# ladnlav/OFDM-course

Hardware: AMD Instinct MI355X
Metric: OFDM sym/s full Task-5 RX (Nfft=2048, 64-QAM, OMP) (higher is better)
Workload: dtype f32; 1 GPU; M: Nfft=2048 Tg=256 N_carrier=512 comb=4 (128 pilots, K=128) 64QAM OMP(6 taps) Noise(20 dB) -> 6-tap channel (the reference's order), frames of 14 symbols; frames_per_gpu=20480

## Files before the change

### ofdm-course_amd/csrc/chain_fast_core.hpp

```cpp
#pragma once
#include <cstdlib>
#include <map>
#include <utility>
#include <vector>
#include <type_traits>

#include "demap_core.hpp"
#include "fft_core.hpp"

namespace ofdm {

constexpr int FAST_MAXT = 32;

__device__ __forceinline__ void wave_sync() {
  __builtin_amdgcn_fence(__ATOMIC_RELEASE, "wavefront");
  __builtin_amdgcn_wave_barrier();
  __builtin_amdgcn_fence(__ATOMIC_ACQUIRE, "wavefront");
}

constexpr int WAVE_LDS_ELEMS = 512 + 64;

constexpr int WAVE_TW_ELEMS = 2 * 7 * 64;

template <typename T, int NW>
__device__ __forceinline__ void wave_tw_fill(cx<T>* __restrict__ twl, const cx<T>* __restrict__ tw) {
  for (int i = threadIdx.x; i < WAVE_TW_ELEMS; i += 64 * NW) {
    const int pass = i / 448, r = i - pass * 448, t = r / 64 + 1, l = r & 63;
    twl[i] = pass == 0 ? tw[(t * (l & 7) * 8) * NW] : tw[(t * l) * NW];
  }
}

template <typename T>
__device__ __forceinline__ void dft8_first2(cx<T> (&v)[8]) {
  const T h = T(0.70710678118654752440084436210485);
  const cx<T> a0 = v[0] + v[4], a1 = v[1] + v[5], a2 = v[2] + v[6], a3 = v[3] + v[7];
  const cx<T> b0 = v[0] - v[4];
  cx<T> b1 = v[1] - v[5], b2 = v[2] - v[6], b3 = v[3] - v[7];
  b1 = mk<T>((b1.x + b1.y) * h, (b1.y - b1.x) * h);
  b2 = mk<T>(b2.y, -b2.x);
  b3 = mk<T>((b3.y - b3.x) * h, (-b3.x - b3.y) * h);
  v[0] = (a0 + a2) + (a1 + a3);
  v[1] = (b0 + b2) + (b1 + b3);
}

template <int STRIDE, bool ASM>
__device__ __forceinline__ void lds_read8(cx<float> (&v)[8], const cx<float>* base) {
  if constexpr (ASM) {
    const unsigned a = (unsigned)(uintptr_t)base;
    unsigned long long r0, r1, r2, r3, r4, r5, r6, r7;
    asm volatile(
        "ds_read_b64 %0, %8 offset:%9\n\t"
        "ds_read_b64 %1, %8 offset:%10\n\t"
        "ds_read_b64 %2, %8 offset:%11\n\t"
        "ds_read_b64 %3, %8 offset:%12\n\t"
        "ds_read_b64 %4, %8 offset:%13\n\t"
        "ds_read_b64 %5, %8 offset:%14\n\t"
        "ds_read_b64 %6, %8 offset:%15\n\t"
        "ds_read_b64 %7, %8 offset:%16\n\t"
        "s_waitcnt lgkmcnt(0)"
        : "=&v"(r0), "=&v"(r1), "=&v"(r2), "=&v"(r3), "=&v"(r4), "=&v"(r5), "=&v"(r6), "=&v"(r7)
        : "v"(a), "n"(0 * STRIDE * 8), "n"(1 * STRIDE * 8), "n"(2 * STRIDE * 8), "n"(3 * STRIDE * 8),
          "n"(4 * STRIDE * 8), "n"(5 * STRIDE * 8), "n"(6 * STRIDE * 8), "n"(7 * STRIDE * 8)
        : "memory");
    const unsigned long long r[8] = {r0, r1, r2, r3, r4, r5, r6, r7};
#pragma unroll
    for (int e = 0; e < 8; ++e) {
      v[e].x = __uint_as_float((unsigned)r[e]);
      v[e].y = __uint_as_float((unsigned)(r[e] >> 32));
    }
  } else {
#pragma unroll
    for (int e = 0; e < 8; ++e) v[e] = base[STRIDE * e];
  }
}
template <int STRIDE, bool ASM>
__device__ __forceinline__ void lds_read8(cx<double> (&v)[8], const cx<double>* base) {
#pragma unroll
  for (int e = 0; e < 8; ++e) v[e] = base[STRIDE * e];
}

template <typename T, bool PRUNE2, bool TWB_REG = true, bool ASMRD = false>
__device__ __forceinline__ void wave_fft512(cx<T> (&v)[8], int lane, const cx<T> (&twb)[7],
                                            const cx<T>* __restrict__ twl, cx<T>* __restrict__ lw) {
  cx<T>* const sa = lw + 72 * (lane >> 3) + (lane & 3) + 36 * ((lane >> 2) & 1);
  cx<T>* const ga1 = lw + ((lane >> 3) & 3) + 36 * (lane >> 5) + 4 * (lane & 7);
  cx<T>* const sb = lw + 72 * (lane >> 3) + (lane & 7);
  cx<T>* const ga2 = lw + lane;
  dft8<T, false>(v[0], v[1], v[2], v[3], v[4], v[5], v[6], v[7]);
#pragma unroll
  for (int t = 0; t < 8; ++t) sa[4 * t] = v[t];
  wave_sync();
  lds_read8<72, ASMRD>(v, ga1);
  wave_sync();
#pragma unroll
  for (int t = 1; t < 8; ++t) v[t] = v[t] * (TWB_REG ? twb[t - 1] : twl[(t - 1) * 64 + lane]);
  dft8<T, false>(v[0], v[1], v[2], v[3], v[4], v[5], v[6], v[7]);
#pragma unroll
  for (int t = 0; t < 8; ++t) sb[8 * t] = v[t];
  wave_sync();
  lds_read8<72, ASMRD>(v, ga2);
  wave_sync();
#pragma unroll
  for (int t = 1; t < 8; ++t) v[t] = v[t] * twl[448 + (t - 1) * 64 + lane];
  if constexpr (PRUNE2) dft8_first2<T>(v);
  else dft8<T, false>(v[0], v[1], v[2], v[3], v[4], v[5], v[6], v[7]);
}

template <typename T, int NW>
struct DifTw {
  cx<T> w[NW > 1 ? (8 / NW) * (NW - 1) : 1];
};

template <typename T, int NW>
__device__ __forceinline__ void dif_tw_init(DifTw<T, NW>& d, int gid, const cx<T>* __restrict__ tw) {
  if constexpr (NW > 1) {
    constexpr int BPT = 8 / NW;
#pragma unroll
    for (int b = 0; b < BPT; ++b)
#pragma unroll
      for (int s = 1; s < NW; ++s) d.w[b * (NW - 1) + (s - 1)] = tw[(gid * BPT + b) * s];
  }
}

template <typename T, int NW>
__device__ __forceinline__ void frame_load(cx<T> (&v)[8], const cx<T>* __restrict__ src ,
                                           int gid, int lane) {
  if constexpr (NW == 1) {
#pragma unroll
    for (int e = 0; e < 8; ++e) v[e] = nt_load(src + lane + 64 * e);
  } else {
    constexpr int BPT = 8 / NW;
#pragma unroll
    for (int t = 0; t < NW; ++t)
#pragma unroll
      for (int b = 0; b < BPT; ++b) v[b * NW + t] = nt_load(src + gid * BPT + b + 512 * t);
  }
}

template <typename T, int NW>
__device__ __forceinline__ void dif_stage(cx<T> (&v)[8], const DifTw<T, NW>& d) {
  if constexpr (NW > 1) {
// ... 415 lines not shown
  const float* d_sb_w;
  const int32_t* d_sb_c0;
  void** ws_v;
  int64_t* ws_v_frames;
  void** ws_h;
  void** ws_x;
  int64_t* ws_x_elems;
  int data_mod4;
  uint32_t descr;
};

template <typename T>
int fast_params_prepare(const FastPlanView& pv, const void* tw, int64_t n_frames, FastParams<T>& P);
template <typename T>
int omp_batch_run(const FastParams<T>& P, int64_t n_frames);

template <typename T>
int eq_demap_run(const FastPlanView& pv, const FastParams<T>& P, const cx<T>* xk, int x_stride, bool hext, int64_t n_frames,
                 void* bits, const void* ref, void* errs, void* h_out, void* idx_out, const double* fine_est, int time_desync,
                 int freq_desync, int mer_skip = 0,
                 double* mer_sums = nullptr );

int mmse_build_operator(const c64* h, int64_t n_h, double snr_db, const int32_t* pilot_loc, int np, int n_carrier,
                        int m_pad, std::vector<c64>& wt, std::vector<c64>* mt_out = nullptr, int np_pad = 0,
                        std::vector<double>* sop_out = nullptr);
void mmse_band_spline(const std::vector<double>& sop, int nc, int np, std::vector<float>& w, std::vector<int32_t>& c0, int& bw, int& span);
int spline_band_run(const float* sb_w, const int32_t* sb_c0, int bw, int span, const void* v, void* hout, int np, int n_carrier,
                    int64_t n_frames);
bool mmse_factored_usable(int np, int np_pad);
int mmse_factored_run(const void* mt, int np_pad, const float* sb_w, const int32_t* sb_c0, int bw, int span, const void* y, void* v,
                      void* hout, int np, int n_carrier, int64_t n_frames);
template <typename T>
int mmse_apply_run(const void* wt, const void* y, void* hout, int np, int m_pad, int n_carrier, int64_t n_frames);

template <typename T>
inline int mmse_stage_run(const FastPlanView& pv, const FastParams<T>& P, int64_t n_frames) {
  if constexpr (std::is_same<T, float>::value) {
    if (pv.d_mt && mmse_factored_usable(pv.np, pv.np_pad)) {
      int64_t& cap = *pv.ws_v_frames;
      if (!*pv.ws_v || cap < n_frames) {
        OFDM_HIP(hipStreamSynchronize(ctx().stream));
        if (*pv.ws_v) { (void)hipFree(*pv.ws_v); *pv.ws_v = nullptr; }
        OFDM_HIP(hipMalloc(pv.ws_v, sizeof(cx<float>) * (size_t)pv.np * n_frames));
        cap = n_frames;
      }
      return mmse_factored_run(pv.d_mt, pv.np_pad, pv.d_sb_w, pv.d_sb_c0, pv.sb_bw, pv.sb_span, P.ypil, *pv.ws_v, *pv.ws_h, pv.np,
                               pv.n_carrier, n_frames);
    }
  }
  return mmse_apply_run<T>(pv.d_wt, P.ypil, *pv.ws_h, pv.np, pv.m_pad, pv.n_carrier, n_frames);
}

bool chain_wave_supported(const FastPlanView& pv);
int chain_wave_symbols_run(const FastPlanView& pv, const FastParams<float>& P, const void* rx, int64_t n_frames, void* bits,
                           const void* ref, void* errs, void* h_out, void* idx_out, double* mer = nullptr );

bool chain_coop_supported(const FastPlanView& pv);
int chain_coop_symbols_run(const FastPlanView& pv, const FastParams<float>& P, const void* rx, int64_t n_frames, void* bits,
                           const void* ref, void* errs, void* h_out, void* idx_out, double* mer = nullptr );

template <typename T>
int pilot_omp_run(const FastParams<T>& P, int nfft, bool prune2, int lg_up, const void* rx, int64_t n_frames);

}
```

### ofdm-course_amd/csrc/ofdm_chain_fast.hip

```cpp
#include "chain_fast_core.hpp"
#include "omp_wave_core.hpp"

namespace ofdm {

template <typename T, int NW, bool PRUNE2>
__global__ __launch_bounds__(64 * NW, sizeof(T) == 4 ? (PRUNE2 ? 4 : 3) : 2) void rx_pilot_kernel(FastParams<T> P, const cx<T>* __restrict__ rx,
                                                           int64_t n_frames) {
  constexpr int N = 512 * NW;
  constexpr int NOUT = PRUNE2 ? 2 : 8;
  __shared__ cx<T> lwv[NW * WAVE_LDS_ELEMS];
  __shared__ cx<T> twl[WAVE_TW_ELEMS];
  cx<T>* const ex = lwv;
  const int wave = threadIdx.x >> 6, lane = threadIdx.x & 63, gid = threadIdx.x;
  DifTw<T, NW> dt;
  wave_tw_fill<T, NW>(twl, P.tw);
  dif_tw_init<T, NW>(dt, gid, P.tw);
  cx<T> twb[7];
#pragma unroll
  for (int t = 1; t < 8; ++t) twb[t - 1] = P.tw[(t * (lane & 7) * 8) * NW];
  __syncthreads();
  int kk[NOUT], pp[NOUT];
#pragma unroll
  for (int t = 0; t < NOUT; ++t) {
    kk[t] = NW * (lane + 64 * t) + wave;
// ... 338 lines not shown
  P.tap_idx = (int32_t*)*pv.ws_tapidx; P.tap_x = (c64*)*pv.ws_tapx;
  const bool mmse = pv.d_wt != nullptr;
  if (mmse && !*pv.ws_h) {
    OFDM_HIP(hipStreamSynchronize(ctx().stream));
    OFDM_HIP(hipMalloc(pv.ws_h, sizeof(cx<T>) * (size_t)pv.n_carrier * *pv.ws_frames));
  }
  P.h_in = mmse ? (const cx<T>*)*pv.ws_h : nullptr;
  P.descr = pv.descr;
  return OFDM_OK;
}
template int fast_params_prepare<float>(const FastPlanView&, const void*, int64_t, FastParams<float>&);
template int fast_params_prepare<double>(const FastPlanView&, const void*, int64_t, FastParams<double>&);

template <typename T>
int omp_batch_run(const FastParams<T>& P, int64_t n_frames) {
  hipStream_t st = ctx().stream;
  const bool by_fft = P.comb_m == 2048 && P.np <= 2048 && P.k_atoms <= 2048 && !getenv("OFDM_OMP_NO_FFT");
  const OmpLayout lay = omp_layout<T>(P.np, P.k_atoms, P.taps, by_fft ? fft_lds_elems(2048) : 0);
  OFDM_ARG(lay.total <= 150 * 1024, "rx_chain_task5: OMP stage needs %u bytes of LDS", lay.total);
  const unsigned grid = cdiv_u(n_frames, 4 * lay.fpw);
  const bool mfma = std::is_same<T, float>::value && (P.k_atoms % 16 == 0) && (P.np % 4 == 0) && !getenv("OFDM_OMP_NO_MFMA");
  auto launch = [&](auto kern, const void* twm) -> int {
    OFDM_HIP(hipFuncSetAttribute((const void*)kern, hipFuncAttributeMaxDynamicSharedMemorySize, (int)lay.total));
    hipLaunchKernelGGL(kern, dim3(grid), dim3(256), lay.total, st, P, lay, n_frames, (const cx<T>*)twm);
    return OFDM_OK;
  };
  if (by_fft) {
    const void* twm = nullptr;
    OFDM_TRY(get_twiddles(2048, std::is_same<T, double>::value, &twm));
    OFDM_TRY(launch(omp_batch_kernel<T, false, 2048>, twm));
  } else if (mfma) {
    if constexpr (std::is_same<T, float>::value) OFDM_TRY(launch(omp_batch_kernel<T, true>, nullptr));
  } else {
    OFDM_TRY(launch(omp_batch_kernel<T, false>, nullptr));
  }
  return check_launch("omp_batch_kernel");
}
template int omp_batch_run<float>(const FastParams<float>&, int64_t);
template int omp_batch_run<double>(const FastParams<double>&, int64_t);

template <typename T, int NW, bool PRUNE2>
static int launch_fast(const FastPlanView& pv, const void* tw, const void* rx, int64_t n_frames, void* bits,
                       const void* ref, void* errs, void* h_out, void* idx_out, double* mer) {
  FastParams<T> P;
  OFDM_TRY(fast_params_prepare<T>(pv, tw, n_frames, P));
  const bool mmse = pv.d_wt != nullptr;
  DemapTable<T> tab;
  fill_demap_table<T>(*pv.dict, *pv.cinfo, tab);
  const int ncu = ctx().num_cu;
  hipStream_t st = ctx().stream;
  if (pv.ev) OFDM_HIP(hipEventRecord(pv.ev[0], st));
  const bool fused = !mmse && pv.comb_lg_up >= 0 && pv.taps <= OMP_RT && pv.k_atoms <= 512 && !getenv("OFDM_FAST_UNFUSED");
  if (pv.fused_out) *pv.fused_out = fused ? 1 : 0;
  if (fused) {
    OFDM_TRY(pilot_omp_run<T>(P, 512 * NW, PRUNE2, pv.comb_lg_up, rx, n_frames));
    if (pv.ev) OFDM_HIP(hipEventRecord(pv.ev[1], st));
  } else {
    {
      const unsigned grid = (unsigned)std::min<int64_t>(n_frames, (int64_t)ncu * std::max(1, 16 / NW));
      hipLaunchKernelGGL((rx_pilot_kernel<T, NW, PRUNE2>), dim3(grid), dim3(64 * NW), 0, st, P, (const cx<T>*)rx, n_frames);
      OFDM_TRY(check_launch("rx_pilot_kernel"));
    }
    if (pv.ev) OFDM_HIP(hipEventRecord(pv.ev[1], st));
    if (mmse) {
      OFDM_TRY(mmse_stage_run<T>(pv, P, n_frames));
    } else {
      OFDM_TRY(omp_batch_run<T>(P, n_frames));
    }
  }
  if (pv.ev && !fused) OFDM_HIP(hipEventRecord(pv.ev[2], st));
  if constexpr (std::is_same<T, float>::value && NW == 4 && PRUNE2) {
    if (chain_wave_supported(pv) && !(mer && getenv("OFDM_WAVE_EXACT_SLICER"))) {
      OFDM_TRY(chain_wave_symbols_run(pv, P, rx, n_frames, bits, ref, errs, h_out, idx_out, mer));
      if (pv.ev) OFDM_HIP(hipEventRecord(pv.ev[3], st));
      return OFDM_OK;
    }
  }
  {
    constexpr int N = 512 * NW;
    const size_t dyn = sizeof(cx<T>) * ((size_t)NW * WAVE_LDS_ELEMS + WAVE_TW_ELEMS) +
                       (((size_t)pv.nd * pv.n_symb + 31) & ~size_t(31));
    OFDM_ARG(dyn <= 150 * 1024, "rx_chain_task5: symbol stage needs %zu bytes of LDS", dyn);
    auto launch = [&](auto kern, auto... mer_arg) -> int {
      int per_cu = resident_blocks_per_cu((const void*)kern, 64 * NW, dyn);
      if (const char* e = getenv("OFDM_FAST_WG_PER_CU")) per_cu = std::max(1, atoi(e));
      const unsigned grid = (unsigned)std::min<int64_t>(n_frames, (int64_t)ncu * per_cu);
      hipLaunchKernelGGL(kern, dim3(grid), dim3(64 * NW), dyn, st, P, (const cx<T>*)rx, n_frames, (uint32_t*)bits,
                         (const uint32_t*)ref, (uint32_t*)errs, (cx<T>*)h_out, (int32_t*)idx_out, tab, mer_arg...);
      return OFDM_OK;
    };
    const int ba = pv.cinfo->kind == 1 ? pv.cinfo->bits_per_axis : 0;
    if (mer) {
      const MerSums ms{mer};
      switch (ba) {
        case 2: OFDM_TRY(mmse ? launch(rx_symbols_kernel<T, NW, PRUNE2, 2, true, MerSums>, ms)
                              : launch(rx_symbols_kernel<T, NW, PRUNE2, 2, false, MerSums>, ms)); break;
        case 3: OFDM_TRY(mmse ? launch(rx_symbols_kernel<T, NW, PRUNE2, 3, true, MerSums>, ms)
                              : launch(rx_symbols_kernel<T, NW, PRUNE2, 3, false, MerSums>, ms)); break;
        case 4: OFDM_TRY(mmse ? launch(rx_symbols_kernel<T, NW, PRUNE2, 4, true, MerSums>, ms)
                              : launch(rx_symbols_kernel<T, NW, PRUNE2, 4, false, MerSums>, ms)); break;
        default: OFDM_TRY(mmse ? launch(rx_symbols_kernel<T, NW, PRUNE2, 0, true, MerSums>, ms)
                               : launch(rx_symbols_kernel<T, NW, PRUNE2, 0, false, MerSums>, ms)); break;
      }
    } else if (mmse) {
      switch (ba) {
        case 2: OFDM_TRY(launch(rx_symbols_kernel<T, NW, PRUNE2, 2, true>)); break;
        case 3: OFDM_TRY(launch(rx_symbols_kernel<T, NW, PRUNE2, 3, true>)); break;
        case 4: OFDM_TRY(launch(rx_symbols_kernel<T, NW, PRUNE2, 4, true>)); break;
        default: OFDM_TRY(launch(rx_symbols_kernel<T, NW, PRUNE2, 0, true>)); break;
      }
    } else {
      switch (ba) {
        case 2: OFDM_TRY(launch(rx_symbols_kernel<T, NW, PRUNE2, 2>)); break;
        case 3: OFDM_TRY(launch(rx_symbols_kernel<T, NW, PRUNE2, 3>)); break;
        case 4: OFDM_TRY(launch(rx_symbols_kernel<T, NW, PRUNE2, 4>)); break;
        default: OFDM_TRY(launch(rx_symbols_kernel<T, NW, PRUNE2, 0>)); break;
      }
    }
    OFDM_TRY(check_launch("rx_symbols_kernel"));
  }
  if (pv.ev) OFDM_HIP(hipEventRecord(pv.ev[3], st));
  return OFDM_OK;
}

template <typename T>
// ... 26 lines not shown
```

### ofdm-course_amd/csrc/ofdm_chain_pilot.hip

```cpp
#include <algorithm>

#include "chain_fast_core.hpp"

namespace ofdm {

template <typename T, int NW, bool PRUNE2, int RT>
__global__ __launch_bounds__(64 * NW) void rx_pilot_omp_kernel(FastParams<T> P, int lg_up, int fpw, int ystride,
                                                               const cx<T>* __restrict__ rx, int64_t n_frames) {
  constexpr int N = 512 * NW;
  constexpr int NOUT = PRUNE2 ? 2 : 8;
  extern __shared__ __attribute__((aligned(16))) unsigned char smem[];
  cx<T>* lwv = (cx<T>*)smem;
  cx<T>* const ex = lwv;
  cx<T>* twl = lwv + NW * WAVE_LDS_ELEMS;
  cx<T>* gl = twl + WAVE_TW_ELEMS;
  cx<T>* ybuf = gl + P.k_atoms;
  const int wave = threadIdx.x >> 6, lane = threadIdx.x & 63, gid = threadIdx.x;
  const int np = P.np, K = P.k_atoms;
  const int G = NW * fpw;
  wave_tw_fill<T, NW>(twl, P.tw);
  for (int i = gid; i < K; i += 64 * NW) gl[i] = mk<T>((T)P.gram[i].x, (T)P.gram[i].y);
  __syncthreads();
  const int64_t L = (int64_t)(N + P.t_guard) * P.n_symb;
  const int64_t n_groups = (n_frames + G - 1) / G;
  const int up_mask = (1 << lg_up) - 1;
  const int LPF = 64 / fpw, grp = lane / LPF, sl = lane - grp * LPF;
  for (int64_t g = blockIdx.x; g < n_groups; g += gridDim.x) {
    int opq = 0;
    asm volatile("" : "+v"(opq));
    DifTw<T, NW> dt;
    dif_tw_init<T, NW>(dt, gid + opq, P.tw);
    cx<T> twb[7];
#pragma unroll
    for (int t = 1; t < 8; ++t) twb[t - 1] = P.tw[(t * ((lane + opq) & 7) * 8) * NW];
    int kk[NOUT], pp[NOUT];
#pragma unroll
    for (int t = 0; t < NOUT; ++t) {
      kk[t] = NW * (lane + 64 * t) + wave + opq;
      pp[t] = kk[t] < P.n_carrier ? (int)P.prole[kk[t]] : -1;
    }
    cx<T> v[8], nx[8];
    frame_load<T, NW>(nx, rx + g * G * L + P.t_guard, gid, lane);
    for (int j = 0; j < G; ++j) {
      const int64_t f = g * G + j;
      if (f >= n_frames) break;
#pragma unroll
      for (int e = 0; e < 8; ++e) v[e] = nx[e];
      if (j + 1 < G && f + 1 < n_frames) frame_load<T, NW>(nx, rx + (f + 1) * L + P.t_guard, gid, lane);
      if constexpr (NW > 1) {
        dif_stage<T, NW>(v, dt);
        __syncthreads();
        dif_scatter<T, NW>(v, gid, ex);
        __syncthreads();
        dif_gather<T>(v, wave, lane, ex);
      }
      wave_fft512<T, PRUNE2>(v, lane, twb, twl, lwv + wave * WAVE_LDS_ELEMS);
#pragma unroll
      for (int t = 0; t < NOUT; ++t) {
        if (kk[t] < P.n_carrier) {
          P.stash[f * P.n_carrier + kk[t]] = v[t];
          if (pp[t] >= 0) ybuf[j * ystride + pp[t]] = cdiv(v[t], P.pilots[pp[t]]);
        }
      }
    }
    __syncthreads();
    const int64_t fw0 = g * G + wave * fpw;
    if (fw0 < n_frames) {
      cx<T>* const lw = lwv + wave * WAVE_LDS_ELEMS;
      cx<T>* const yw = ybuf + wave * fpw * ystride;
      cx<T>* const yg = yw + grp * ystride;
      double ynorm = 0;
      for (int p = sl; p < np; p += LPF) ynorm += (double)yg[p].x * yg[p].x + (double)yg[p].y * yg[p].y;
      for (int off = LPF >> 1; off > 0; off >>= 1) ynorm += __shfl_xor(ynorm, off, 64);
      for (int j = 0; j < fpw; ++j) {
        if (fw0 + j >= n_frames) break;
        cx<T>* const yf = yw + j * ystride;
        cx<T> c[8];
#pragma unroll
        for (int e = 0; e < 8; ++e) {
          const int i = lane + 64 * e, p = i >> lg_up;
          c[e] = ((i & up_mask) == 0 && p < np) ? conj(yf[p]) : mk<T>(0, 0);
        }
        wave_fft512<T, false>(c, lane, twb, twl, lw);
#pragma unroll
        for (int t = 0; t < 8; ++t)
          if (lane + 64 * t < K) yf[lane + 64 * t] = conj(c[t]);
      }
      wave_sync();
      omp_frame_reg<T, RT>(P, yg, gl, K, P.taps, LPF, sl, fw0 + grp < n_frames, ynorm, fw0 + grp);
    }
    __syncthreads();
  }
}

template <typename T, int NW, bool PRUNE2, int RT>
static int pilot_omp_launch(const FastParams<T>& P, int lg_up, const void* rx, int64_t n_frames) {
  const int ystride = std::max(P.np, P.k_atoms);
  int fpw = 4;
  if (const char* e = getenv("OFDM_PILOT_FPW")) { const int v = atoi(e); if (v == 1 || v == 2 || v == 4 || v == 8) fpw = v; }
  while (fpw > 1 && sizeof(cx<T>) * (size_t)NW * fpw * ystride > 8 * 1024) fpw >>= 1;
  const size_t dyn = sizeof(cx<T>) * ((size_t)NW * WAVE_LDS_ELEMS + WAVE_TW_ELEMS + P.k_atoms + (size_t)NW * fpw * ystride);
  OFDM_ARG(dyn <= 150 * 1024, "rx_chain_task5: pilot stage needs %zu bytes of LDS", dyn);
  auto kern = rx_pilot_omp_kernel<T, NW, PRUNE2, RT>;
  const int per_cu = resident_blocks_per_cu((const void*)kern, 64 * NW, dyn);
  const int64_t groups = (n_frames + NW * fpw - 1) / (NW * fpw);
  const unsigned grid = (unsigned)std::min<int64_t>(groups, (int64_t)ctx().num_cu * per_cu);
  hipLaunchKernelGGL(kern, dim3(grid), dim3(64 * NW), dyn, ctx().stream, P, lg_up, fpw, ystride, (const cx<T>*)rx, n_frames);
  return check_launch("rx_pilot_omp_kernel");
}

template <typename T, int NW, bool PRUNE2>
static int pilot_omp_taps(const FastParams<T>& P, int lg_up, const void* rx, int64_t n_frames) {
  if (P.taps <= 2) return pilot_omp_launch<T, NW, PRUNE2, 2>(P, lg_up, rx, n_frames);
  if (P.taps <= 4) return pilot_omp_launch<T, NW, PRUNE2, 4>(P, lg_up, rx, n_frames);
  if (P.taps <= 6) return pilot_omp_launch<T, NW, PRUNE2, 6>(P, lg_up, rx, n_frames);
  return pilot_omp_launch<T, NW, PRUNE2, 8>(P, lg_up, rx, n_frames);
}

template <typename T>
int pilot_omp_run(const FastParams<T>& P, int nfft, bool prune2, int lg_up, const void* rx, int64_t n_frames) {
  OFDM_ARG(P.taps <= OMP_RT && P.k_atoms <= 512 && lg_up >= 0, "rx_chain_task5: pilot stage called outside its domain");
#define PILOT_CALL(NWV)                                                              \
  return prune2 ? pilot_omp_taps<T, NWV, true>(P, lg_up, rx, n_frames)               \
                : pilot_omp_taps<T, NWV, false>(P, lg_up, rx, n_frames)
  switch (nfft / 512) {
    case 1: PILOT_CALL(1);
    case 2: PILOT_CALL(2);
    case 4: PILOT_CALL(4);
    case 8: PILOT_CALL(8);
  }
#undef PILOT_CALL
  set_error("rx_chain_task5(pilot stage): unsupported Nfft %d", nfft);
  return OFDM_ERR_UNSUPPORTED;
}

template int pilot_omp_run<float>(const FastParams<float>&, int, bool, int, const void*, int64_t);
template int pilot_omp_run<double>(const FastParams<double>&, int, bool, int, const void*, int64_t);

}
```

### ofdm-course_amd/csrc/ofdm_chain_wave.hip

```cpp
#include <algorithm>
#include <type_traits>

#include "chain_fast_core.hpp"

namespace ofdm {

constexpr int WV_N = 2048;
constexpr int WV_TR_ELEMS = 576;
constexpr int WV_TW_ROWS = 31;
constexpr int WV_WPB = 4;

constexpr unsigned WV_OFF_TW = 0, WV_OFF_TWB = 8 * 64 * WV_TW_ROWS, WV_OFF_DD = WV_OFF_TWB + 8 * 64 * 7;
constexpr unsigned WV_OFF_LUT = WV_OFF_DD + 8 * 64 * 4;
constexpr unsigned WV_OFF_WAVE = WV_OFF_LUT + 256;
constexpr unsigned WV_TRASH_OFF = 8 * WV_TR_ELEMS, WV_DESCR_OFF = WV_TRASH_OFF + 8 * 64, WV_CODES_OFF = WV_DESCR_OFF + 16;
struct WaveLayout {
  unsigned wave_bytes, total;
  int cb;
};

__device__ __forceinline__ cx<float> w32(int m) {
  constexpr float C[9] = {1.0f, 0.98078528040323044913f, 0.92387953251128675613f, 0.83146961230254523708f,
                          0.70710678118654752440f, 0.55557023301960222474f, 0.38268343236508977173f,
                          0.19509032201612826785f, 0.0f};
  m &= 31;
  const int q = m >> 3, r = m & 7;
  const float c = C[r], s = C[8 - r];
  switch (q) {
    case 0: return mk<float>(c, -s);
    case 1: return mk<float>(-s, -c);
    case 2: return mk<float>(-c, s);
    default: return mk<float>(s, c);
  }
}

__host__ __device__ constexpr int wv_reg(int L, int j0, int m) { return L == 0 ? j0 + 4 * m : 4 * j0 + 16 * (m >> 2) + (m & 3); }

template <int BA, int SL>
__device__ __forceinline__ int slice_wave(const DemapTable<float>& tab, const float* lut, cx<float> z) {
  if constexpr (SL == 1 && BA >= 2) return demap_square_lut<float, BA>(tab, lut, z);
  else if constexpr (SL == 2 && BA >= 2) return demap_square_arith<BA>(tab, z);
  else return slice_symbol<float, BA, true>(tab, z);
}

template <int BA, bool HEXT, int WPB = WV_WPB, int ABL = 0, bool WBUF = true, int LUT = 2, int SKIP = 0, bool DESCR = false,
          typename... Mer>
__global__ __launch_bounds__(64 * WPB, sizeof...(Mer) ? 2 : (WPB == 8 ? 4 : 3)) void rx_symbols_wave_kernel(FastParams<float> P, WaveLayout lay,
                                                                  const cx<float>* __restrict__ rx, int64_t n_frames,
                                                                  uint32_t* __restrict__ bits_out,
                                                                  const uint32_t* __restrict__ ref_bits,
                                                                  uint32_t* __restrict__ errors_out,
                                                                  cx<float>* __restrict__ h_out,
                                                                  int32_t* __restrict__ index_out, DemapTable<float> tab,
                                                                  Mer... mer) {
  using T = float;
  constexpr bool MER = sizeof...(Mer) == 1;
  extern __shared__ __attribute__((aligned(16))) unsigned char smem[];
  const int lane = threadIdx.x & 63;
  const int wave = __builtin_amdgcn_readfirstlane(threadIdx.x >> 6);
  const int n_waves_wg = blockDim.x >> 6;
  const unsigned lane8 = 8u * lane;
  auto tw32_at = [&](int row) { return *(const cx<T>*)(smem + WV_OFF_TW + 512 * row + lane8); };
  auto twbl_at = [&](int row) { return *(const cx<T>*)(smem + WV_OFF_TWB + 512 * row + lane8); };
  {
    cx<T>* const tw32 = (cx<T>*)(smem + WV_OFF_TW);
    cx<T>* const twbl = (cx<T>*)(smem + WV_OFF_TWB);
    for (int i = threadIdx.x; i < WV_TW_ROWS * 64; i += blockDim.x) {
      const int kj = i / 64 + 1, l = i & 63;
      tw32[i] = P.tw[(kj * l) & (WV_N - 1)];
    }
    for (int i = threadIdx.x; i < 7 * 64; i += blockDim.x) {
      const int t = i / 64 + 1, l = i & 63;
      twbl[i] = P.tw[t * (l & 7) * 32];
    }
  }
  const int nd = P.nd, taps = P.taps, n_symb = P.n_symb, n_carrier = P.n_carrier;
  const int Lsym = WV_N + P.t_guard;
  const int64_t Lframe = (int64_t)Lsym * n_symb;
  const int CB = lay.cb;
  const int c_out = lane >> 3, ka_out = lane & 7;
  auto kk_of = [&](int t) { return 32 * (ka_out + 8 * (t & 1)) + (t >> 1) + 4 * c_out; };
  if (wave == 0) {
#pragma unroll
    for (int r = 0; r < 4; ++r) {
      const int k0 = kk_of(2 * r), k1 = kk_of(2 * r + 1);
      const unsigned d0 = k0 < n_carrier ? (unsigned)(unsigned short)P.drole[k0] : 0xffffu;
      const unsigned d1 = k1 < n_carrier ? (unsigned)(unsigned short)P.drole[k1] : 0xffffu;
      *(unsigned*)(smem + WV_OFF_DD + 512 * r + lane8) = d0 | (d1 << 16);
    }
  }
  const T* const lut = (const T*)(smem + WV_OFF_LUT);
  if constexpr (BA >= 2) demap_lut_fill<T, BA>(tab, (T*)(smem + WV_OFF_LUT), threadIdx.x);
  double* const mer_out = mer_sums_of(mer...);
  const T* mt = nullptr;
  if constexpr (MER) {
    __shared__ T mer_tab[32];
    mer_tab_fill<T>(tab, mer_tab, threadIdx.x);
    mt = mer_tab;
  }
  __syncthreads();
  const unsigned wbase = WV_OFF_WAVE + (unsigned)wave * lay.wave_bytes;
  unsigned char* const trl = smem + wbase + lane8;
  uint8_t* const codes = smem + wbase + WV_CODES_OFF;
  auto code_ptr = [&](uint8_t* base, int t) {
    const unsigned d = (*(const unsigned*)(smem + WV_OFF_DD + 512 * (t >> 1) + lane8) >> (16 * (t & 1))) & 0xffffu;
    return d == 0xffffu ? (uint8_t*)(trl + WV_TRASH_OFF) : base + d;
  };
  auto mer_take = [&](int t, int code, cx<T> z, double& s1, double& s2) __attribute__((always_inline)) {
    const unsigned d = (*(const unsigned*)(smem + WV_OFF_DD + 512 * (t >> 1) + lane8) >> (16 * (t & 1))) & 0xffffu;
    if (d != 0xffffu) mer_add(mer_ideal<T, BA>(tab, mt, code), z, s1, s2);
  };
  cx<T>* const t1w = (cx<T>*)trl;
  cx<T>* const t1r = (cx<T>*)(smem + wbase) + 72 * (lane >> 3) + (lane & 7);
  cx<T>* const t2w = (cx<T>*)(smem + wbase) + 65 * (lane & 7) + 8 * (lane >> 3);
  cx<T>* const t2r = (cx<T>*)trl;

  const int64_t wave_id = (int64_t)blockIdx.x * n_waves_wg + wave, n_waves = (int64_t)gridDim.x * n_waves_wg;
  cx<T> v[32];
  cx<T> w[8];
  if (wave_id < n_frames && n_symb > 1) {
    const cx<T>* src = rx + wave_id * Lframe + Lsym + P.t_guard + lane;
#pragma unroll
    for (int r = 0; r < (WBUF ? 3 : 4); ++r)
#pragma unroll
      for (int c = 0; c < 8; ++c) v[4 * c + r] = nt_load(src + 64 * (4 * c + r));
    if constexpr (WBUF) {
#pragma unroll
      for (int c = 0; c < 8; ++c) w[c] = nt_load(src + 64 * (4 * c + 3));
    }
  }
  auto do_frame = [&](auto SC, int64_t f) __attribute__((always_inline)) {
    constexpr int S0 = decltype(SC)::value;
    const cx<T>* frx = rx + f * Lframe;
    const int64_t fnext = f + n_waves;
    cx<T> geq[8];
    if constexpr (HEXT) {
#pragma unroll
      for (int t = 0; t < 8; ++t) {
        geq[t] = mk<T>(0, 0);
        if (kk_of(t) < n_carrier) {
          const cx<T> H = P.h_in[f * n_carrier + kk_of(t)];
          if (h_out) h_out[f * n_carrier + kk_of(t)] = H;
          geq[t] = cdiv(mk<T>(1, 0), H);
        }
      }
    } else {
      double hr[8], hi[8];
#pragma unroll
      for (int t = 0; t < 8; ++t) hr[t] = hi[t] = 0.0;
      for (int q = 0; q < taps; ++q) {
        const int idx = P.tap_idx[f * taps + q];
        const c64 x = P.tap_x[f * taps + q];
        if (index_out && lane == 0) index_out[f * taps + q] = idx + 1;
        const int id0 = idx < 0 ? 0 : idx;
#pragma unroll
        for (int t = 0; t < 8; ++t) {
          const int e = (id0 * kk_of(t)) & (WV_N - 1);
          const float turns = (float)e * (1.0f / (float)WV_N);
          const float ws = __builtin_amdgcn_sinf(turns), wc = __builtin_amdgcn_cosf(turns);
          hr[t] += x.x * (double)wc + x.y * (double)ws;
          hi[t] += x.y * (double)wc - x.x * (double)ws;
        }
      }
#pragma unroll
      for (int t = 0; t < 8; ++t) {
        geq[t] = mk<T>(0, 0);
        if (kk_of(t) < n_carrier) {
          const cx<T> H = mk<T>((T)hr[t], (T)hi[t]);
          if (h_out) h_out[f * n_carrier + kk_of(t)] = H;
          geq[t] = cdiv(mk<T>(1, 0), H);
        }
      }
    }
    double s1 = 0, s2 = 0;
#pragma unroll
    for (int t = 0; t < 8; ++t) {
      const cx<T> z = (kk_of(t) < n_carrier ? P.stash[f * n_carrier + kk_of(t)] : mk<T>(0, 0)) * geq[t];
      const int code = slice_wave<BA, LUT>(tab, lut, z);
      *code_ptr(codes, t) = (uint8_t)code;
      if constexpr (MER) mer_take(t, code, z, s1, s2);
    }
    unsigned err = 0;
    int slot = 1;
    int64_t code0 = 0;
    uint32_t* const dslot = (uint32_t*)(smem + wbase + WV_DESCR_OFF);
    if constexpr (DESCR) { if (lane == 0) *dslot = P.descr; }
    auto symbol = [&](auto LC, int s) __attribute__((always_inline)) {
      constexpr int L = decltype(LC)::value;
      const cx<T>* nsrc = frx + (int64_t)s * Lsym + P.t_guard + lane;
      if (s + 1 < n_symb) nsrc += Lsym;
      else if (fnext < n_frames) nsrc = rx + fnext * Lframe + Lsym + P.t_guard + lane;
      uint8_t* const cslot = codes + slot * nd;
      {
#pragma unroll
        for (int j0 = 0; j0 < 4; ++j0) {
          if (WBUF && j0 == 3) {
            dft8<T, false>(w[0], w[1], w[2], w[3], w[4], w[5], w[6], w[7]);
#pragma unroll
            for (int ka = 0; ka < 8; ++ka) v[wv_reg(L, 3, ka)] = w[ka];
            if constexpr (ABL != 1) {
#pragma unroll
              for (int m = 0; m < 8; ++m) w[m] = nt_load(nsrc + 64 * (3 + 4 * m));
            }
          } else {
            dft8<T, false>(v[wv_reg(L, j0, 0)], v[wv_reg(L, j0, 1)], v[wv_reg(L, j0, 2)], v[wv_reg(L, j0, 3)], v[wv_reg(L, j0, 4)],
                           v[wv_reg(L, j0, 5)], v[wv_reg(L, j0, 6)], v[wv_reg(L, j0, 7)]);
          }
          if (j0 > 0) {
#pragma unroll
            for (int ka = 1; ka < 8; ++ka)
              if (!((SKIP >> (ka & 3)) & 1)) v[wv_reg(L, j0, ka)] = v[wv_reg(L, j0, ka)] * w32(j0 * ka);
          }
        }
#pragma unroll
        for (int ka = 0; ka < 8; ++ka)
          if (!((SKIP >> (ka & 3)) & 1))
            dft4<T, false>(v[wv_reg(L, 0, ka)], v[wv_reg(L, 1, ka)], v[wv_reg(L, 2, ka)], v[wv_reg(L, 3, ka)]);
#pragma unroll
        for (int r = 0; r < 4; ++r) {
          const bool skip = (SKIP >> r) & 1;
          cx<T> z_keep[8];
          if (!skip) {
#pragma unroll
            for (int c = 0; c < 8; ++c) {
              const int kj = r + 4 * c, ka = r + 4 * (c & 1), kb = c >> 1;
              const cx<T> z = kj == 0 ? v[wv_reg(L, kb, ka)] : v[wv_reg(L, kb, ka)] * tw32_at(kj - 1);
              t1w[72 * c] = z;
              z_keep[c] = z;
            }
// ... 55 lines not shown
    for (int s = 1; s < n_symb; s += 2) {
      symbol(std::integral_constant<int, S0>{}, s);
      if (s + 1 < n_symb) symbol(std::integral_constant<int, 1 - S0>{}, s + 1);
    }
    if (n_symb == 1) {
      const int n_codes = nd, pad_to = (n_codes + 31) & ~31;
      if (lane < pad_to - n_codes) codes[n_codes + lane] = 0;
      wave_sync();
      err += pack_frame_t<2 * BA, DESCR>(codes, n_codes, P.bps, P.frame_words, bits_out ? bits_out + f * P.frame_words : nullptr,
                                         ref_bits ? ref_bits + f * P.frame_words : nullptr, lane, 64, P.descr);
      wave_sync();
    }
    if (ref_bits && errors_out) {
      for (int off = 32; off > 0; off >>= 1) err += __shfl_xor(err, off, 64);
      if (lane == 0) errors_out[f] = err;
    }
    if constexpr (MER) {
      mer_wave_sum(s1, s2);
      if (lane == 0) *(double2*)(mer_out + 2 * f) = make_double2(s1, s2);
    }
  };
  const bool odd = ((n_symb - 1) & 1) != 0;
  for (int64_t f = wave_id; f < n_frames;) {
    do_frame(std::integral_constant<int, 0>{}, f);
    f += n_waves;
    if (odd) {
      if (f >= n_frames) break;
      do_frame(std::integral_constant<int, 1>{}, f);
      f += n_waves;
    }
  }
}

static bool wave_layout(int nd, int n_symb, int wpb, WaveLayout& lay) {
  int cb = 1;
  while ((cb * nd) % 32 != 0) ++cb;
  const int unit = cb;
  while (cb * nd < 1920 && cb < n_symb) cb += unit;
  if (cb >= n_symb) cb = n_symb;
  const unsigned codes_bytes = (unsigned)(((size_t)cb * nd + 31 + 32) & ~size_t(31));
  if (codes_bytes > 6144) return false;
  lay.cb = cb;
  lay.wave_bytes = (WV_CODES_OFF + codes_bytes + 15) & ~15u;
  lay.total = WV_OFF_WAVE + (unsigned)wpb * lay.wave_bytes;
  return lay.total <= (wpb == 8 ? 78u : 52u) * 1024;
}

bool chain_wave_supported(const FastPlanView& pv) {
  if (getenv("OFDM_FAST_NO_WAVE")) return false;
  if ((pv.descr & DESCR_ON) && pv.d_wt != nullptr) return false;
  if (pv.f64 || pv.nfft != WV_N || pv.n_carrier > WV_N / 4 || pv.taps > FAST_MAXT) return false;
  WaveLayout lay;
  return wave_layout(pv.nd, pv.n_symb, 4, lay) && wave_layout(pv.nd, pv.n_symb, 8, lay);
}

int chain_wave_symbols_run(const FastPlanView& pv, const FastParams<float>& P, const void* rx, int64_t n_frames, void* bits,
                           const void* ref, void* errs, void* h_out, void* idx_out, double* mer) {
  const int wpb = WV_WPB;
  WaveLayout lay;
  OFDM_ARG(wave_layout(pv.nd, pv.n_symb, wpb, lay), "rx_chain_task5(wave): frame does not fit the wave-per-frame stage");
  DemapTable<float> tab;
  fill_demap_table<float>(*pv.dict, *pv.cinfo, tab);
  const bool mmse = pv.d_wt != nullptr;
  auto launch = [&](auto kern, auto... mer_arg) -> int {
    int per_cu = resident_blocks_per_cu((const void*)kern, 64 * wpb, lay.total);
    if (const char* e = getenv("OFDM_WAVE_WG_PER_CU")) per_cu = std::max(1, atoi(e));
    const int64_t want = (n_frames + wpb - 1) / wpb;
    const unsigned grid = (unsigned)std::min<int64_t>(want, (int64_t)ctx().num_cu * per_cu);
    hipLaunchKernelGGL(kern, dim3(grid), dim3(64 * wpb), lay.total, ctx().stream, P, lay, (const cx<float>*)rx, n_frames,
                       (uint32_t*)bits, (const uint32_t*)ref, (uint32_t*)errs, (cx<float>*)h_out, (int32_t*)idx_out, tab,
                       mer_arg...);
    return OFDM_OK;
  };
  const int ba = pv.cinfo->kind == 1 ? pv.cinfo->bits_per_axis : 0;
  const bool exact = getenv("OFDM_WAVE_EXACT_SLICER") != nullptr;
  const bool skip0 = (pv.data_mod4 & 15) == 14 && !getenv("OFDM_WAVE_NO_SKIP");
  const bool skip02 = (pv.data_mod4 & 15) == 10 && !getenv("OFDM_WAVE_NO_SKIP");
#define WAVE_CASE(BAV, HX)                                                                \
  if (exact) OFDM_TRY(launch(rx_symbols_wave_kernel<BAV, HX, 4, 0, true, 0>));            \
  else if (skip0) OFDM_TRY(launch(rx_symbols_wave_kernel<BAV, HX, 4, 0, true, 2, 1>));    \
  else if (skip02) OFDM_TRY(launch(rx_symbols_wave_kernel<BAV, HX, 4, 0, true, 2, 5>));   \
  else OFDM_TRY(launch(rx_symbols_wave_kernel<BAV, HX, 4>))
#define WAVE_CASE_D(BAV)                                                                            \
  if (exact) OFDM_TRY(launch(rx_symbols_wave_kernel<BAV, false, 4, 0, true, 0, 0, true>));          \
  else if (skip0) OFDM_TRY(launch(rx_symbols_wave_kernel<BAV, false, 4, 0, true, 2, 1, true>));     \
  else if (skip02) OFDM_TRY(launch(rx_symbols_wave_kernel<BAV, false, 4, 0, true, 2, 5, true>));    \
  else OFDM_TRY(launch(rx_symbols_wave_kernel<BAV, false, 4, 0, true, 2, 0, true>))
#define WAVE_CASE_M(BAV, HX)                                                                                         \
  if (skip0) OFDM_TRY(launch(rx_symbols_wave_kernel<BAV, HX, 4, 0, true, 2, 1, false, MerSums>, MerSums{mer}));      \
  else if (skip02) OFDM_TRY(launch(rx_symbols_wave_kernel<BAV, HX, 4, 0, true, 2, 5, false, MerSums>, MerSums{mer})); \
  else OFDM_TRY(launch(rx_symbols_wave_kernel<BAV, HX, 4, 0, true, 2, 0, false, MerSums>, MerSums{mer}))
  if (mer) {
    OFDM_ARG(!exact && !(P.descr & DESCR_ON), "rx_chain_task5(wave): no MER variant of the exact-slicer / DeScrambler forms");
    switch (ba) {
      case 2: if (mmse) { WAVE_CASE_M(2, true); } else { WAVE_CASE_M(2, false); } break;
      case 3: if (mmse) { WAVE_CASE_M(3, true); } else { WAVE_CASE_M(3, false); } break;
      case 4: if (mmse) { WAVE_CASE_M(4, true); } else { WAVE_CASE_M(4, false); } break;
      default: if (mmse) { WAVE_CASE_M(0, true); } else { WAVE_CASE_M(0, false); } break;
    }
  } else if (P.descr & DESCR_ON) {
    OFDM_ARG(!mmse, "rx_chain_task5(wave): the DeScrambler variant exists in OMP mode only");
    switch (ba) {
      case 2: WAVE_CASE_D(2); break;
      case 3: WAVE_CASE_D(3); break;
      case 4: WAVE_CASE_D(4); break;
      default: WAVE_CASE_D(0); break;
    }
  } else if (mmse) {
    switch (ba) {
      case 2: WAVE_CASE(2, true); break;
      case 3: WAVE_CASE(3, true); break;
      case 4: WAVE_CASE(4, true); break;
      default: WAVE_CASE(0, true); break;
    }
  } else {
    switch (ba) {
      case 2: WAVE_CASE(2, false); break;
      case 3:
#ifdef OFDM_DIAG
        if (getenv("OFDM_WAVE_ABL")) { OFDM_TRY(launch(rx_symbols_wave_kernel<3, false, 4, 1>)); break; }
#endif
        WAVE_CASE(3, false);
        break;
      case 4: WAVE_CASE(4, false); break;
      default: WAVE_CASE(0, false); break;
    }
  }
#undef WAVE_CASE
#undef WAVE_CASE_D
#undef WAVE_CASE_M
// ... 5 lines not shown
```

Before: 311.6 million OFDM symbols/s.

## Prune pilot-stage stash writes, zero-input FFT pass, and skipped-carrier channel work

The pilot OMP kernel now skips writing stashed subcarriers whose residue class the wave symbol stage will never read (pilot/null positions), saving global stores. When pilots only fill the first 128 bins, the correlation FFT uses a specialized leading DFT8 pass that assumes only two non-zero inputs and writes back only the needed outputs. The wave kernel also skips channel-from-taps evaluation and slicing for skipped carriers and uses a cheaper reciprocal. This adds template variants and env switches, and relies on the skip mask staying consistent between the two kernels.

```diff
diff --git a/ofdm-course_amd/csrc/chain_fast_core.hpp b/ofdm-course_amd/csrc/chain_fast_core.hpp
--- a/ofdm-course_amd/csrc/chain_fast_core.hpp
+++ b/ofdm-course_amd/csrc/chain_fast_core.hpp
@@ -41,6 +41,22 @@
   b3 = mk<T>((b3.y - b3.x) * h, (-b3.x - b3.y) * h);
   v[0] = (a0 + a2) + (a1 + a3);
   v[1] = (b0 + b2) + (b1 + b3);
+}
+
+template <typename T>
+__device__ __forceinline__ void dft8_lead2(cx<T> (&v)[8]) {
+  const T h = T(0.70710678118654752440084436210485);
+  const cx<T> a0 = v[0], a1 = v[1];
+  T wx = (a1.x + a1.y) * h, wy = (a1.y - a1.x) * h;
+  asm("" : "+v"(wx), "+v"(wy));
+  v[0] = mk<T>(a0.x + a1.x, a0.y + a1.y);
+  v[1] = mk<T>(a0.x + wx, a0.y + wy);
+  v[2] = mk<T>(a0.x + a1.y, a0.y - a1.x);
+  v[3] = mk<T>(a0.x + wy, a0.y - wx);
+  v[4] = mk<T>(a0.x - a1.x, a0.y - a1.y);
+  v[5] = mk<T>(a0.x - wx, a0.y - wy);
+  v[6] = mk<T>(a0.x - a1.y, a0.y + a1.x);
+  v[7] = mk<T>(a0.x - wy, a0.y + wx);
 }
 
 template <int STRIDE, bool ASM>
@@ -79,14 +95,16 @@
   for (int e = 0; e < 8; ++e) v[e] = base[STRIDE * e];
 }
 
-template <typename T, bool PRUNE2, bool TWB_REG = true, bool ASMRD = false>
+template <typename T, bool PRUNE2, bool TWB_REG = true, bool ASMRD = false, int NIN = 8>
 __device__ __forceinline__ void wave_fft512(cx<T> (&v)[8], int lane, const cx<T> (&twb)[7],
                                             const cx<T>* __restrict__ twl, cx<T>* __restrict__ lw) {
+  static_assert(NIN == 2 || NIN == 8, "leading pass: two or eight non-zero registers");
   cx<T>* const sa = lw + 72 * (lane >> 3) + (lane & 3) + 36 * ((lane >> 2) & 1);
   cx<T>* const ga1 = lw + ((lane >> 3) & 3) + 36 * (lane >> 5) + 4 * (lane & 7);
   cx<T>* const sb = lw + 72 * (lane >> 3) + (lane & 7);
   cx<T>* const ga2 = lw + lane;
-  dft8<T, false>(v[0], v[1], v[2], v[3], v[4], v[5], v[6], v[7]);
+  if constexpr (NIN == 2) dft8_lead2<T>(v);
+  else dft8<T, false>(v[0], v[1], v[2], v[3], v[4], v[5], v[6], v[7]);
 #pragma unroll
   for (int t = 0; t < 8; ++t) sa[4 * t] = v[t];
   wave_sync();
@@ -608,6 +626,7 @@
 }
 
 bool chain_wave_supported(const FastPlanView& pv);
+int chain_wave_skip_mask(const FastPlanView& pv);
 int chain_wave_symbols_run(const FastPlanView& pv, const FastParams<float>& P, const void* rx, int64_t n_frames, void* bits,
                            const void* ref, void* errs, void* h_out, void* idx_out, double* mer = nullptr );
 
@@ -616,6 +635,6 @@
                            const void* ref, void* errs, void* h_out, void* idx_out, double* mer = nullptr );
 
 template <typename T>
-int pilot_omp_run(const FastParams<T>& P, int nfft, bool prune2, int lg_up, const void* rx, int64_t n_frames);
-
-}
+int pilot_omp_run(const FastParams<T>& P, int nfft, bool prune2, int lg_up, const void* rx, int64_t n_frames, int stash_skip);
+
+}
diff --git a/ofdm-course_amd/csrc/ofdm_chain_fast.hip b/ofdm-course_amd/csrc/ofdm_chain_fast.hip
--- a/ofdm-course_amd/csrc/ofdm_chain_fast.hip
+++ b/ofdm-course_amd/csrc/ofdm_chain_fast.hip
@@ -414,8 +414,12 @@
   if (pv.ev) OFDM_HIP(hipEventRecord(pv.ev[0], st));
   const bool fused = !mmse && pv.comb_lg_up >= 0 && pv.taps <= OMP_RT && pv.k_atoms <= 512 && !getenv("OFDM_FAST_UNFUSED");
   if (pv.fused_out) *pv.fused_out = fused ? 1 : 0;
+  bool wave = false;
+  if constexpr (std::is_same<T, float>::value && NW == 4 && PRUNE2)
+    wave = chain_wave_supported(pv) && !(mer && getenv("OFDM_WAVE_EXACT_SLICER"));
   if (fused) {
-    OFDM_TRY(pilot_omp_run<T>(P, 512 * NW, PRUNE2, pv.comb_lg_up, rx, n_frames));
+    const int stash_skip = wave ? chain_wave_skip_mask(pv) : 0;
+    OFDM_TRY(pilot_omp_run<T>(P, 512 * NW, PRUNE2, pv.comb_lg_up, rx, n_frames, stash_skip));
     if (pv.ev) OFDM_HIP(hipEventRecord(pv.ev[1], st));
   } else {
     {
@@ -432,7 +436,7 @@
   }
   if (pv.ev && !fused) OFDM_HIP(hipEventRecord(pv.ev[2], st));
   if constexpr (std::is_same<T, float>::value && NW == 4 && PRUNE2) {
-    if (chain_wave_supported(pv) && !(mer && getenv("OFDM_WAVE_EXACT_SLICER"))) {
+    if (wave) {
       OFDM_TRY(chain_wave_symbols_run(pv, P, rx, n_frames, bits, ref, errs, h_out, idx_out, mer));
       if (pv.ev) OFDM_HIP(hipEventRecord(pv.ev[3], st));
       return OFDM_OK;
diff --git a/ofdm-course_amd/csrc/ofdm_chain_pilot.hip b/ofdm-course_amd/csrc/ofdm_chain_pilot.hip
--- a/ofdm-course_amd/csrc/ofdm_chain_pilot.hip
+++ b/ofdm-course_amd/csrc/ofdm_chain_pilot.hip
@@ -4,8 +4,8 @@
 
 namespace ofdm {
 
-template <typename T, int NW, bool PRUNE2, int RT>
-__global__ __launch_bounds__(64 * NW) void rx_pilot_omp_kernel(FastParams<T> P, int lg_up, int fpw, int ystride,
+template <typename T, int NW, bool PRUNE2, int RT, bool C0P>
+__global__ __launch_bounds__(64 * NW) void rx_pilot_omp_kernel(FastParams<T> P, int lg_up, int fpw, int ystride, int stash_skip,
                                                                const cx<T>* __restrict__ rx, int64_t n_frames) {
   constexpr int N = 512 * NW;
   constexpr int NOUT = PRUNE2 ? 2 : 8;
@@ -58,7 +58,7 @@
 #pragma unroll
       for (int t = 0; t < NOUT; ++t) {
         if (kk[t] < P.n_carrier) {
-          P.stash[f * P.n_carrier + kk[t]] = v[t];
+          if (!((stash_skip >> (kk[t] & 3)) & 1)) P.stash[f * P.n_carrier + kk[t]] = v[t];
           if (pp[t] >= 0) ybuf[j * ystride + pp[t]] = cdiv(v[t], P.pilots[pp[t]]);
         }
       }
@@ -75,15 +75,16 @@
       for (int j = 0; j < fpw; ++j) {
         if (fw0 + j >= n_frames) break;
         cx<T>* const yf = yw + j * ystride;
+        constexpr int NC = C0P ? 2 : 8;
         cx<T> c[8];
 #pragma unroll
         for (int e = 0; e < 8; ++e) {
           const int i = lane + 64 * e, p = i >> lg_up;
-          c[e] = ((i & up_mask) == 0 && p < np) ? conj(yf[p]) : mk<T>(0, 0);
+          c[e] = (e < NC && (i & up_mask) == 0 && p < np) ? conj(yf[p]) : mk<T>(0, 0);
         }
-        wave_fft512<T, false>(c, lane, twb, twl, lw);
+        wave_fft512<T, C0P, true, false, NC>(c, lane, twb, twl, lw);
 #pragma unroll
-        for (int t = 0; t < 8; ++t)
+        for (int t = 0; t < NC; ++t)
           if (lane + 64 * t < K) yf[lane + 64 * t] = conj(c[t]);
       }
       wave_sync();
@@ -93,36 +94,41 @@
   }
 }
 
-template <typename T, int NW, bool PRUNE2, int RT>
-static int pilot_omp_launch(const FastParams<T>& P, int lg_up, const void* rx, int64_t n_frames) {
+template <typename T, int NW, bool PRUNE2, int RT, bool C0P>
+static int pilot_omp_launch(const FastParams<T>& P, int lg_up, const void* rx, int64_t n_frames, int stash_skip) {
   const int ystride = std::max(P.np, P.k_atoms);
   int fpw = 4;
   if (const char* e = getenv("OFDM_PILOT_FPW")) { const int v = atoi(e); if (v == 1 || v == 2 || v == 4 || v == 8) fpw = v; }
   while (fpw > 1 && sizeof(cx<T>) * (size_t)NW * fpw * ystride > 8 * 1024) fpw >>= 1;
   const size_t dyn = sizeof(cx<T>) * ((size_t)NW * WAVE_LDS_ELEMS + WAVE_TW_ELEMS + P.k_atoms + (size_t)NW * fpw * ystride);
   OFDM_ARG(dyn <= 150 * 1024, "rx_chain_task5: pilot stage needs %zu bytes of LDS", dyn);
-  auto kern = rx_pilot_omp_kernel<T, NW, PRUNE2, RT>;
+  auto kern = rx_pilot_omp_kernel<T, NW, PRUNE2, RT, C0P>;
   const int per_cu = resident_blocks_per_cu((const void*)kern, 64 * NW, dyn);
   const int64_t groups = (n_frames + NW * fpw - 1) / (NW * fpw);
   const unsigned grid = (unsigned)std::min<int64_t>(groups, (int64_t)ctx().num_cu * per_cu);
-  hipLaunchKernelGGL(kern, dim3(grid), dim3(64 * NW), dyn, ctx().stream, P, lg_up, fpw, ystride, (const cx<T>*)rx, n_frames);
+  hipLaunchKernelGGL(kern, dim3(grid), dim3(64 * NW), dyn, ctx().stream, P, lg_up, fpw, ystride, stash_skip, (const cx<T>*)rx,
+                     n_frames);
   return check_launch("rx_pilot_omp_kernel");
 }
 
-template <typename T, int NW, bool PRUNE2>
-static int pilot_omp_taps(const FastParams<T>& P, int lg_up, const void* rx, int64_t n_frames) {
-  if (P.taps <= 2) return pilot_omp_launch<T, NW, PRUNE2, 2>(P, lg_up, rx, n_frames);
-  if (P.taps <= 4) return pilot_omp_launch<T, NW, PRUNE2, 4>(P, lg_up, rx, n_frames);
-  if (P.taps <= 6) return pilot_omp_launch<T, NW, PRUNE2, 6>(P, lg_up, rx, n_frames);
-  return pilot_omp_launch<T, NW, PRUNE2, 8>(P, lg_up, rx, n_frames);
+template <typename T, int NW, bool PRUNE2, bool C0P>
+static int pilot_omp_taps(const FastParams<T>& P, int lg_up, const void* rx, int64_t n_frames, int stash_skip) {
+  if (P.taps <= 2) return pilot_omp_launch<T, NW, PRUNE2, 2, C0P>(P, lg_up, rx, n_frames, stash_skip);
+  if (P.taps <= 4) return pilot_omp_launch<T, NW, PRUNE2, 4, C0P>(P, lg_up, rx, n_frames, stash_skip);
+  if (P.taps <= 6) return pilot_omp_launch<T, NW, PRUNE2, 6, C0P>(P, lg_up, rx, n_frames, stash_skip);
+  return pilot_omp_launch<T, NW, PRUNE2, 8, C0P>(P, lg_up, rx, n_frames, stash_skip);
 }
 
 template <typename T>
-int pilot_omp_run(const FastParams<T>& P, int nfft, bool prune2, int lg_up, const void* rx, int64_t n_frames) {
+int pilot_omp_run(const FastParams<T>& P, int nfft, bool prune2, int lg_up, const void* rx, int64_t n_frames, int stash_skip) {
   OFDM_ARG(P.taps <= OMP_RT && P.k_atoms <= 512 && lg_up >= 0, "rx_chain_task5: pilot stage called outside its domain");
-#define PILOT_CALL(NWV)                                                              \
-  return prune2 ? pilot_omp_taps<T, NWV, true>(P, lg_up, rx, n_frames)               \
-                : pilot_omp_taps<T, NWV, false>(P, lg_up, rx, n_frames)
+  if (getenv("OFDM_PILOT_FULL_STASH")) stash_skip = 0;
+  const bool c0p = (((int64_t)P.np - 1) << lg_up) < 128 && P.k_atoms <= 128 && !getenv("OFDM_PILOT_NO_C0_PRUNE");
+#define PILOT_CALL(NWV)                                                                                  \
+  return prune2 ? (c0p ? pilot_omp_taps<T, NWV, true, true>(P, lg_up, rx, n_frames, stash_skip)          \
+                       : pilot_omp_taps<T, NWV, true, false>(P, lg_up, rx, n_frames, stash_skip))        \
+                : (c0p ? pilot_omp_taps<T, NWV, false, true>(P, lg_up, rx, n_frames, stash_skip)         \
+                       : pilot_omp_taps<T, NWV, false, false>(P, lg_up, rx, n_frames, stash_skip))
   switch (nfft / 512) {
     case 1: PILOT_CALL(1);
     case 2: PILOT_CALL(2);
@@ -134,7 +140,7 @@
   return OFDM_ERR_UNSUPPORTED;
 }
 
-template int pilot_omp_run<float>(const FastParams<float>&, int, bool, int, const void*, int64_t);
-template int pilot_omp_run<double>(const FastParams<double>&, int, bool, int, const void*, int64_t);
+template int pilot_omp_run<float>(const FastParams<float>&, int, bool, int, const void*, int64_t, int);
+template int pilot_omp_run<double>(const FastParams<double>&, int, bool, int, const void*, int64_t, int);
 
 }
diff --git a/ofdm-course_amd/csrc/ofdm_chain_wave.hip b/ofdm-course_amd/csrc/ofdm_chain_wave.hip
--- a/ofdm-course_amd/csrc/ofdm_chain_wave.hip
+++ b/ofdm-course_amd/csrc/ofdm_chain_wave.hip
@@ -35,6 +35,12 @@
 }
 
 __host__ __device__ constexpr int wv_reg(int L, int j0, int m) { return L == 0 ? j0 + 4 * m : 4 * j0 + 16 * (m >> 2) + (m & 3); }
+
+__device__ __forceinline__ cx<float> recip_h(cx<float> H) {
+  const float d = 1.0f / __builtin_fmaf(H.x, H.x, H.y * H.y);
+  const cx<float> one = mk<float>(1, 0);
+  return mk<float>((one.x * H.x + one.y * H.y) * d, (one.y * H.x - one.x * H.y) * d);
+}
 
 template <int BA, int SL>
 __device__ __forceinline__ int slice_wave(const DemapTable<float>& tab, const float* lut, cx<float> z) {
@@ -134,47 +140,56 @@
     const cx<T>* frx = rx + f * Lframe;
     const int64_t fnext = f + n_waves;
     cx<T> geq[8];
+    auto skipped = [](int t) { return ((SKIP >> (t >> 1)) & 1) != 0; };
     if constexpr (HEXT) {
 #pragma unroll
       for (int t = 0; t < 8; ++t) {
         geq[t] = mk<T>(0, 0);
-        if (kk_of(t) < n_carrier) {
+        if (kk_of(t) < n_carrier && (!skipped(t) || h_out)) {
           const cx<T> H = P.h_in[f * n_carrier + kk_of(t)];
           if (h_out) h_out[f * n_carrier + kk_of(t)] = H;
-          geq[t] = cdiv(mk<T>(1, 0), H);
+          geq[t] = recip_h(H);
         }
       }
     } else {
-      double hr[8], hi[8];
-#pragma unroll
-      for (int t = 0; t < 8; ++t) hr[t] = hi[t] = 0.0;
-      for (int q = 0; q < taps; ++q) {
-        const int idx = P.tap_idx[f * taps + q];
-        const c64 x = P.tap_x[f * taps + q];
-        if (index_out && lane == 0) index_out[f * taps + q] = idx + 1;
-        const int id0 = idx < 0 ? 0 : idx;
+      auto h_from_taps = [&](auto ALLC) __attribute__((always_inline)) {
+        constexpr bool ALL = decltype(ALLC)::value;
+        double hr[8], hi[8];
+#pragma unroll
+        for (int t = 0; t < 8; ++t) hr[t] = hi[t] = 0.0;
+        for (int q = 0; q < taps; ++q) {
+          const int idx = P.tap_idx[f * taps + q];
+          const c64 x = P.tap_x[f * taps + q];
+          if (index_out && lane == 0) index_out[f * taps + q] = idx + 1;
+          const int id0 = idx < 0 ? 0 : idx;
+#pragma unroll
+          for (int t = 0; t < 8; ++t) {
+            if (!ALL && skipped(t)) continue;
+            const int e = (id0 * kk_of(t)) & (WV_N - 1);
+            const float turns = (float)e * (1.0f / (float)WV_N);
+            const float ws = __builtin_amdgcn_sinf(turns), wc = __builtin_amdgcn_cosf(turns);
+            hr[t] += x.x * (double)wc + x.y * (double)ws;
+            hi[t] += x.y * (double)wc - x.x * (double)ws;
+          }
+        }
 #pragma unroll
         for (int t = 0; t < 8; ++t) {
-          const int e = (id0 * kk_of(t)) & (WV_N - 1);
-          const float turns = (float)e * (1.0f / (float)WV_N);
-          const float ws = __builtin_amdgcn_sinf(turns), wc = __builtin_amdgcn_cosf(turns);
-          hr[t] += x.x * (double)wc + x.y * (double)ws;
-          hi[t] += x.y * (double)wc - x.x * (double)ws;
-        }
-      }
-#pragma unroll
-      for (int t = 0; t < 8; ++t) {
-        geq[t] = mk<T>(0, 0);
-        if (kk_of(t) < n_carrier) {
-          const cx<T> H = mk<T>((T)hr[t], (T)hi[t]);
-          if (h_out) h_out[f * n_carrier + kk_of(t)] = H;
-          geq[t] = cdiv(mk<T>(1, 0), H);
-        }
-      }
+          geq[t] = mk<T>(0, 0);
+          if (!ALL && skipped(t)) continue;
+          if (kk_of(t) < n_carrier) {
+            const cx<T> H = mk<T>((T)hr[t], (T)hi[t]);
+            if (h_out) h_out[f * n_carrier + kk_of(t)] = H;
+            geq[t] = recip_h(H);
+          }
+        }
+      };
+      if (SKIP == 0 || h_out) h_from_taps(std::true_type{});
+      else h_from_taps(std::false_type{});
     }
     double s1 = 0, s2 = 0;
 #pragma unroll
     for (int t = 0; t < 8; ++t) {
+      if (skipped(t)) continue;
       const cx<T> z = (kk_of(t) < n_carrier ? P.stash[f * n_carrier + kk_of(t)] : mk<T>(0, 0)) * geq[t];
       const int code = slice_wave<BA, LUT>(tab, lut, z);
       *code_ptr(codes, t) = (uint8_t)code;
@@ -336,6 +351,13 @@
   if (pv.f64 || pv.nfft != WV_N || pv.n_carrier > WV_N / 4 || pv.taps > FAST_MAXT) return false;
   WaveLayout lay;
   return wave_layout(pv.nd, pv.n_symb, 4, lay) && wave_layout(pv.nd, pv.n_symb, 8, lay);
+}
+
+int chain_wave_skip_mask(const FastPlanView& pv) {
+  if (getenv("OFDM_WAVE_NO_SKIP") || getenv("OFDM_WAVE_EXACT_SLICER")) return 0;
+  if ((pv.data_mod4 & 15) == 14) return 1;
+  if ((pv.data_mod4 & 15) == 10) return 5;
+  return 0;
 }
 
 int chain_wave_symbols_run(const FastPlanView& pv, const FastParams<float>& P, const void* rx, int64_t n_frames, void* bits,
@@ -358,8 +380,9 @@
   };
   const int ba = pv.cinfo->kind == 1 ? pv.cinfo->bits_per_axis : 0;
   const bool exact = getenv("OFDM_WAVE_EXACT_SLICER") != nullptr;
-  const bool skip0 = (pv.data_mod4 & 15) == 14 && !getenv("OFDM_WAVE_NO_SKIP");
-  const bool skip02 = (pv.data_mod4 & 15) == 10 && !getenv("OFDM_WAVE_NO_SKIP");
+  const int skip_mask = chain_wave_skip_mask(pv);
+  const bool skip0 = skip_mask == 1;
+  const bool skip02 = skip_mask == 5;
 #define WAVE_CASE(BAV, HX)                                                                \
   if (exact) OFDM_TRY(launch(rx_symbols_wave_kernel<BAV, HX, 4, 0, true, 0>));            \
   else if (skip0) OFDM_TRY(launch(rx_symbols_wave_kernel<BAV, HX, 4, 0, true, 2, 1>));    \
```

Result: no change. 314.6 million OFDM symbols/s, median of 6 (+1.0%).
